# pandekan/tomography_alignment

Measured on AMD Instinct MI355X. Metric: sirt_iterations_per_sec, higher is better.
Workload: dtype f32

## Files before the change

### tomography_alignment_amd/csrc/kernels_tile_gather.hip.h

```cpp

#define GTX 8
#define GTY 8
#define GROWS 14
#define GPITCH 68
#ifndef GWAVES
#define GWAVES 4
#endif
#ifndef GPX
#define GPX 8
#define GPY 12
#endif

#define G_DPP(V, CTRL) __builtin_amdgcn_update_dpp(0, (V), (CTRL), 0xf, 0xf, true)
__device__ __forceinline__ int gwave_min_i32(int v)
{
    v = min(v, G_DPP(v, 0xB1));
    v = min(v, G_DPP(v, 0x4E));
    v = min(v, G_DPP(v, 0x141));
    v = min(v, G_DPP(v, 0x140));
    return min(min(__builtin_amdgcn_readlane(v, 0), __builtin_amdgcn_readlane(v, 16)), min(__builtin_amdgcn_readlane(v, 32), __builtin_amdgcn_readlane(v, 48)));
}
__device__ __forceinline__ int gwave_max_i32(int v)
{
    v = max(v, G_DPP(v, 0xB1));
// ... 251 lines not shown
    float4 t = {0.f, 0.f, 0.f, 0.f};
    int ix_lo = 0;
    bool hit = false;
    if (n_grp > 0) {
        G_TABLE(rk, 0, rk)
        __syncthreads();
        float4 tn;
        int ix_lo_n = 0;
        bool hit_n;
        float y0v[GROWS], yedge = 0.f;
        G_SETUP(0, 0, 0)
        hit = hit_n;
        if (hit) G_STAGE(0)
        t = tn; ix_lo = ix_lo_n;
    }
    for (int grp = 0; grp < n_grp; ++grp) {
        const int nbuf = buf == 2 ? 0 : buf + 1;
        if (grp + 1 < n_grp) G_TABLE((grp + 1) * nl + rk, nbuf, rk)
        __syncthreads();
        const int g0 = grp * nl, g1 = min(n_proj, g0 + nl);
        for (int ip = g0; ip < g1; ++ip) {
            float4 tn = t;
            int ix_lo_n = ix_lo;
            bool hit_n = false;
            float y0v[GROWS], yedge = 0.f;
            const bool more = ip + 1 < n_proj;
            if (more) {
                const bool same = ip + 1 < g1;
                const int sbuf = same ? buf : nbuf, sslot = same ? ip + 1 - g0 : 0;
                G_SETUP(ip + 1, sbuf, sslot)
            }
            if (hit) {
                const int i0 = __builtin_bit_cast(int, t.x);
                const float W0 = t.y, W1 = t.z, W2 = t.w;
                const int slot0 = min(max(i0 - ix_lo, 0), GROWS - 3);
                const float4 *q = (const float4 *)__builtin_assume_aligned(wrows + slot0 * GPITCH, 16);
                float4 n0 = q[0], n1 = q[GPITCH / 4], n2 = q[2 * GPITCH / 4];
#pragma unroll
                for (int p = 0; p < 64; p += 4) {
                    const float4 r0 = n0, r1 = n1, r2 = n2;
                    if (p + 4 < 64) { n0 = q[(p + 4) / 4]; n1 = q[(GPITCH + p + 4) / 4]; n2 = q[(2 * GPITCH + p + 4) / 4]; }
                    acc2[p / 2] = W2 * f32x2{r2.x, r2.y} + (W1 * f32x2{r1.x, r1.y} + (W0 * f32x2{r0.x, r0.y} + acc2[p / 2]));
                    acc2[p / 2 + 1] = W2 * f32x2{r2.z, r2.w} + (W1 * f32x2{r1.z, r1.w} + (W0 * f32x2{r0.z, r0.w} + acc2[p / 2 + 1]));
                    __builtin_amdgcn_sched_barrier(0);
                }
            }
            hit = hit_n;
            if (hit) G_STAGE(ip + 1)
            t = tn; ix_lo = ix_lo_n;
        }
        buf = nbuf;
    }
#undef G_TABLE
#undef G_ROW_LOAD
#undef G_SETUP
#undef G_ZLERP
#undef G_STAGE
#undef G_HIT
    if (UPD) {
        if (X < xe && Y < g.ny) {
            const size_t o = ((size_t)X * g.ny + Y) * g.nz + z0;
            gather_update_store<false>(vol + o, upd_v + o, upd_gt ? upd_gt + o : nullptr, acc2, z0, g.nz, positivity, upd_err);
        }
    } else if (zlive && X < xe && Y < g.ny) {
        float *dst = vol + ((size_t)X * g.ny + Y) * g.nz + z0;
        if (z0 + 64 <= g.nz && (g.nz & 3) == 0) {
#pragma unroll
            for (int p = 0; p < 64; p += 4) {
                float4 v = *(float4 *)(dst + p);
                v.x += acc2[p / 2].x; v.y += acc2[p / 2].y; v.z += acc2[p / 2 + 1].x; v.w += acc2[p / 2 + 1].y;
                *(float4 *)(dst + p) = v;
            }
        } else {
#pragma unroll
            for (int p = 0; p < 64; ++p)
                if (z0 + p < g.nz) dst[p] += (p & 1) ? acc2[p / 2].y : acc2[p / 2].x;
        }
    }
}


#define FGROWS 24
#define FG_NONE (1 << 29)

template <int NW, int WALKY>
__device__ __forceinline__ void fwd_gather_flat_body(const GfC *__restrict__ cs, const int *__restrict__ perm, int n_list, unsigned block_id,
                                                     float *__restrict__ proj, const float *__restrict__ vol, const TomoGeomC &g,
                                                     const unsigned char *__restrict__ vflags, const int *__restrict__ zshift,
                                                     float (*rows)[FGROWS * GPITCH], float4 (*wtab)[GWAVES][64], int (*ltab)[GWAVES][64], int *wlive)
{
    static_assert(NW == 3 || NW == 4, "NW");
    constexpr int SW = FGROWS - NW + 1;
    const int lane = threadIdx.x & 63;
    const int wv = __builtin_amdgcn_readfirstlane(threadIdx.x >> 6);
    const int nS = WALKY ? g.ny : g.nx, nL = WALKY ? g.nx : g.ny;
    const uint32_t strideL4 = (WALKY ? (uint32_t)g.ny * (uint32_t)g.nz : (uint32_t)g.nz) * 4u;
    const size_t strideS = WALKY ? (size_t)g.nz : (size_t)g.ny * g.nz;
    const int npg = (n_list + 7) / 8, nrt = (g.ndx + 7) / 8, nzq = (g.nz + 64 * GWAVES - 1) / (64 * GWAVES) + 1;
    const int m_all = npg * nrt, m8 = (m_all + 7) / 8;
    const int slot_id = (int)(block_id >> 3), xcd = (int)(block_id & 7);
    const int zq = slot_id / m8, tile = xcd * m8 + slot_id % m8;
    if (tile >= m_all || zq >= nzq) return;
    const int pg = tile / nrt, rt = tile % nrt;
    const int z0 = (zq * GWAVES + wv - *zshift) * 64;
    bool zlive = z0 >= 0 && z0 < g.nz;
    if (zlive) {
        const int i = z0 + lane;
        zlive = __builtin_amdgcn_ballot_w64(i < g.nz && vflags[i] != 0) != 0;
    }
    if (lane == 0) wlive[wv] = zlive ? 1 : 0;
    __syncthreads();
    int nl = 0, rk = 0;
#pragma unroll
    for (int w = 0; w < GWAVES; ++w) { nl += wlive[w]; rk += w < wv ? wlive[w] : 0; }
#if !defined(__gfx950__) && !defined(__gfx942__) && !defined(__gfx90a__) && defined(__HIP_DEVICE_COMPILE__)
#error "k_fwd_gather_flat: divergent exit before barriers is only known to be safe on gfx9-family targets (s_barrier ignores ended waves)"
#endif
    if (!zlive) return;

    const int ipl = pg * 8 + (lane >> 3), ix = rt * 8 + (lane & 7);
    const int pe = perm[min(ipl, n_list - 1)];
    const bool ray_ok = ipl < n_list && ix < g.ndx && pe >= 0;
    const GfC &c = cs[max(pe, 0)];
    const int64_t fds = WALKY ? c.fdy : c.fdx, fdl = WALKY ? c.fdx : c.fdy;
    const int64_t bs0 = (WALKY ? c.fp0y : c.fp0x) + (int64_t)ix * (WALKY ? c.fuy : c.fux);
    const int64_t bl0 = (WALKY ? c.fp0x : c.fp0y) + (int64_t)ix * (WALKY ? c.fux : c.fuy);
    const float bsf = (float)((double)bs0 * 2.3283064365386963e-10), inv_ds = (float)(4294967296.0 / (double)fds);
    const int n_smp = ray_ok ? c.n : 0;
    const float two_m32 = 2.3283064365386963e-10f;
    const int Zl = z0 + lane;
    const unsigned long long mz = __builtin_amdgcn_ballot_w64(Zl < g.nz);
    const uint32_t o0 = (uint32_t)min(Zl, g.nz - 1) * 4u;
    float *wrows = rows[wv];
    f32x2 acc2[32];
#pragma unroll
    for (int p = 0; p < 32; ++p) acc2[p] = f32x2{0.f, 0.f};

    int s_lo, s_hi;
    {
        const float dsf = (float)((double)fds * 2.3283064365386963e-10), dlf = (float)((double)fdl * 2.3283064365386963e-10);
        const float blf = (float)((double)bl0 * 2.3283064365386963e-10);
        float ja = 0.f, jb = (float)(n_smp - 1);
        if (fabsf(dlf) > 1e-6f) {
            const float ta = (-1.05f - blf) / dlf, tb = ((float)nL + 0.05f - blf) / dlf;
            ja = fmaxf(ja, fminf(ta, tb) - 2.f);
            jb = fminf(jb, fmaxf(ta, tb) + 2.f);
        } else if (!(blf > -1.5f && blf < (float)nL + 0.5f))
            jb = -1.f;
        int lo = FG_NONE, hi = -FG_NONE;
        if (ja <= jb) {
            const float pa = bsf + ja * dsf, pb = bsf + jb * dsf, top = (float)nS + 4.f;
            lo = (int)floorf(fminf(fmaxf(fminf(pa, pb), -4.f), top)) - 2;
            hi = (int)ceilf(fminf(fmaxf(fmaxf(pa, pb), -4.f), top)) + 3;
        }
        s_lo = max(__builtin_amdgcn_readfirstlane(gwave_min_i32(lo)), 0);
        s_hi = min(__builtin_amdgcn_readfirstlane(gwave_max_i32(hi)), nS);
    }
    if (s_lo >= s_hi) return;

#define FG_TABLE(SX, BUF, SLOT)                                                                                            \
    {                                                                                                                      \
        float W[4] = {0.f, 0.f, 0.f, 0.f};                                                                                 \
        int L0 = FG_NONE;                                                                                                  \
        if ((SX) < s_hi) {                                                                                                 \
            const float ta = ((float)((SX) - 1) - bsf) * inv_ds, tb = ((float)((SX) + 1) - bsf) * inv_ds;                  \
            const int j0 = (int)ceilf(fminf(ta, tb) - 5e-3f);                                                              \
            int64_t sx = bs0 + (int64_t)j0 * fds - ((int64_t)(SX) << 32), sl = bl0 + (int64_t)j0 * fdl;                    \
            float wx[3], fl[3];                                                                                            \
            int hl[3];                                                                                                     \
            _Pragma("unroll") for (int mth = 0; mth < 3; ++mth) {                                                          \
                const int hx = (int)(sx >> 32);                                                                            \
                const float fx = (float)(unsigned)sx * two_m32;                                                            \
                float w = hx == -1 ? fx : (hx == 0 ? 1.f - fx : 0.f);                                                      \
                w = (unsigned)(j0 + mth) < (unsigned)n_smp ? w : 0.f;                                                      \
                wx[mth] = w;                                                                                               \
                hl[mth] = (int)(sl >> 32);                                                                                 \
                fl[mth] = (float)(unsigned)sl * two_m32;                                                                   \
                if (w > 0.f) L0 = min(L0, hl[mth]);                                                                        \
                sx += fds; sl += fdl;                                                                                      \
            }                                                                                                              \
            _Pragma("unroll") for (int mth = 0; mth < 3; ++mth) {                                                          \
                const int rel = hl[mth] - L0;                                                                              \
                const float wl1 = wx[mth] * fl[mth], wl0 = wx[mth] - wl1;                                                  \
                _Pragma("unroll") for (int k = 0; k < NW; ++k) W[k] += rel == k ? wl0 : (rel == k - 1 ? wl1 : 0.f);        \
            }                                                                                                              \
            bool any = false;                                                                                              \
            _Pragma("unroll") for (int k = 0; k < NW; ++k) {                                                               \
                W[k] = (unsigned)(L0 + k) < (unsigned)nL ? W[k] : 0.f;                                                     \
                any |= W[k] != 0.f;                                                                                        \
            }                                                                                                              \
            if (!any) L0 = FG_NONE;                                                                                        \
        }                                                                                                                  \
        wtab[BUF][SLOT][lane] = make_float4(W[0], W[1], W[2], W[3]);                                                       \
        ltab[BUF][SLOT][lane] = L0;                                                                                        \
    }
    const uint32_t slab_bytes = (uint32_t)min(WALKY ? (unsigned long long)(g.nx - 1) * strideL4 + (unsigned long long)g.nz * 4ull
                                                    : (unsigned long long)g.ny * g.nz * 4ull, 0xffffffffull);
#define FG_SLAB_RSRC(SX) __builtin_amdgcn_make_buffer_rsrc((void *)(vol + (size_t)(SX) * strideS), 0, (int)slab_bytes, 0x00020000)
#define FG_LINE_LOAD(RS, SOFF) __builtin_bit_cast(float, __builtin_amdgcn_raw_buffer_load_b32((RS), o0, (SOFF), 0))
#define FG_SETUP(SX, BUF, SLOT)                                                                                            \
    {                                                                                                                      \
        tn = wtab[BUF][SLOT][lane];                                                                                        \
        Ln = ltab[BUF][SLOT][lane];                                                                                        \
        Llo_n = __builtin_amdgcn_readfirstlane(gwave_min_i32(Ln));                                                         \
        Lhi_n = __builtin_amdgcn_readfirstlane(gwave_max_i32(Ln == FG_NONE ? -FG_NONE : Ln));                              \
        need_n = 0;                                                                                                        \
        if (Llo_n != FG_NONE) {                                                                                            \
            const __amdgpu_buffer_rsrc_t srs = FG_SLAB_RSRC(SX);                                                           \
            const uint32_t lineoff = (uint32_t)min(max(Llo_n + min(lane, FGROWS - 1), 0), nL - 1) * strideL4;              \
                    \
            need_n = min(Lhi_n - Llo_n + NW, FGROWS);                                                                      \
            _Pragma("unroll") for (int r4 = 0; r4 < FGROWS; r4 += 4)                                                       \
                if (r4 < need_n) {                                                                                         \
                    _Pragma("unroll") for (int r = r4; r < r4 + 4; ++r)                                                    \
                        yv[r] = FG_LINE_LOAD(srs, (uint32_t)__builtin_amdgcn_readlane((int)lineoff, r));                   \
                }                                                                                                          \
        }                                                                                                                  \
    }
#define FG_STAGE                                                                                                           \
    {                                                                                                                      \
        if (mz == ~0ull) {                                                                                                 \
            _Pragma("unroll") for (int r4 = 0; r4 < FGROWS; r4 += 4)                                                       \
                if (r4 < need_n) {                                                                                         \
                    _Pragma("unroll") for (int r = r4; r < r4 + 4; ++r) wrows[r * GPITCH + lane] = yv[r];                  \
                }                                                                                                          \
        } else {                                                                                                           \
            _Pragma("unroll") for (int r4 = 0; r4 < FGROWS; r4 += 4)                                                       \
                if (r4 < need_n) {                                                                                         \
                    _Pragma("unroll") for (int r = r4; r < r4 + 4; ++r) wrows[r * GPITCH + lane] = select_lanes(yv[r], mz); \
                }                                                                                                          \
        }                                                                                                                  \
    }
#define FG_ACCUM(LBASE)                                                                                                    \
    {                                                                                                                      \
        const int rel = L - (LBASE);                                                                                       \
        const bool inw = (unsigned)rel < (unsigned)SW;                                                                     \
        const int slot0 = inw ? rel : 0;                                                                                   \
        const float W0 = inw ? t.x : 0.f, W1 = inw ? t.y : 0.f, W2 = inw ? t.z : 0.f, W3 = inw ? t.w : 0.f;                \
        const float4 *q = (const float4 *)__builtin_assume_aligned(wrows + slot0 * GPITCH, 16);                            \
        float4 n0 = q[0], n1 = q[GPITCH / 4], n2 = q[2 * GPITCH / 4], n3 = {0.f, 0.f, 0.f, 0.f};                           \
        if (NW == 4) n3 = q[3 * GPITCH / 4];                                                                               \
        _Pragma("unroll") for (int p = 0; p < 64; p += 4) {                                                                \
            const float4 r0 = n0, r1 = n1, r2 = n2, r3 = n3;                                                               \
            if (p + 4 < 64) {                                                                                              \
                n0 = q[(p + 4) / 4]; n1 = q[(GPITCH + p + 4) / 4]; n2 = q[(2 * GPITCH + p + 4) / 4];                       \
                if (NW == 4) n3 = q[(3 * GPITCH + p + 4) / 4];                                                             \
            }                                                                                                              \
            f32x2 a = W2 * f32x2{r2.x, r2.y} + (W1 * f32x2{r1.x, r1.y} + (W0 * f32x2{r0.x, r0.y} + acc2[p / 2]));          \
            f32x2 b = W2 * f32x2{r2.z, r2.w} + (W1 * f32x2{r1.z, r1.w} + (W0 * f32x2{r0.z, r0.w} + acc2[p / 2 + 1]));      \
            if (NW == 4) { a = W3 * f32x2{r3.x, r3.y} + a; b = W3 * f32x2{r3.z, r3.w} + b; }                               \
            acc2[p / 2] = a; acc2[p / 2 + 1] = b;                                                                          \
            __builtin_amdgcn_sched_barrier(0);                                                                             \
        }                                                                                                                  \
    }
    const int n_grp = (s_hi - s_lo + nl - 1) / nl;
    int buf = 0;
    FG_TABLE(s_lo + rk, 0, rk)
    __syncthreads();
    float4 t;
    int L, Llo, Lhi;
    {
        float4 tn;
        int Ln, Llo_n, Lhi_n, need_n;
        float yv[FGROWS];
        FG_SETUP(s_lo, 0, 0)
        FG_STAGE
        t = tn; L = Ln; Llo = Llo_n; Lhi = Lhi_n;
    }
    for (int grp = 0; grp < n_grp; ++grp) {
        const int nbuf = buf == 2 ? 0 : buf + 1;
        if (grp + 1 < n_grp) FG_TABLE(s_lo + (grp + 1) * nl + rk, nbuf, rk)
        __syncthreads();
        const int g0 = s_lo + grp * nl, g1 = min(s_hi, g0 + nl);
        for (int sx = g0; sx < g1; ++sx) {
            float4 tn = t;
            int Ln = L, Llo_n = FG_NONE, Lhi_n = 0, need_n = 0;
            float yv[FGROWS];
            if (sx + 1 < s_hi) {
                const bool same = sx + 1 < g1;
                const int sbuf = same ? buf : nbuf, sslot = same ? sx + 1 - g0 : 0;
                FG_SETUP(sx + 1, sbuf, sslot)
            }
            if (Llo != FG_NONE) {
                FG_ACCUM(Llo)
                for (int lb = Llo + SW; lb <= Lhi; lb += SW) {
                    const __amdgpu_buffer_rsrc_t srs = FG_SLAB_RSRC(sx);
                    for (int r = 0; r < FGROWS; r += 4) {
                        float e[4];
#pragma unroll
                        for (int k = 0; k < 4; ++k) e[k] = FG_LINE_LOAD(srs, (uint32_t)min(max(lb + r + k, 0), nL - 1) * strideL4);
#pragma unroll
                        for (int k = 0; k < 4; ++k) wrows[(r + k) * GPITCH + lane] = select_lanes(e[k], mz);
                    }
                    FG_ACCUM(lb)
                }
            }
            FG_STAGE
            t = tn; L = Ln; Llo = Llo_n; Lhi = Lhi_n;
        }
        buf = nbuf;
    }
#undef FG_TABLE
#undef FG_SLAB_RSRC
#undef FG_LINE_LOAD
#undef FG_SETUP
#undef FG_STAGE
#undef FG_ACCUM
    if (!ray_ok) return;
    const int iz0 = z0 - c.zc;
    float *dst = proj + (size_t)c.slot * ((size_t)g.ndx * g.ndz) + (size_t)ix * g.ndz + iz0;
    const float tau = c.tau;
    if (tau == 0.f) {
        if (iz0 >= 0 && iz0 + 64 <= g.ndz && ((iz0 | g.ndz) & 3) == 0) {
#pragma unroll
            for (int p = 0; p < 64; p += 4) *(float4 *)(dst + p) = make_float4(acc2[p / 2].x, acc2[p / 2].y, acc2[p / 2 + 1].x, acc2[p / 2 + 1].y);
        } else {
#pragma unroll
            for (int p = 0; p < 64; ++p)
                if ((unsigned)(iz0 + p) < (unsigned)g.ndz) dst[p] = (p & 1) ? acc2[p / 2].y : acc2[p / 2].x;
        }
    } else {
        const float wfz = 1.f - tau;
#define FG_S(P) (((P) & 1) ? acc2[(P) / 2].y : acc2[(P) / 2].x)
#pragma unroll
        for (int p = 0; p < 63; ++p)
            if ((unsigned)(iz0 + p) < (unsigned)g.ndz) dst[p] = wfz * FG_S(p) + tau * FG_S(p + 1);
        if ((unsigned)(iz0 + 63) < (unsigned)g.ndz) atomicAdd(dst + 63, wfz * FG_S(63));
        if ((unsigned)(iz0 - 1) < (unsigned)g.ndz) atomicAdd(dst - 1, tau * FG_S(0));
#undef FG_S
    }
}

__global__ __launch_bounds__(GWAVES * 64, 3) void k_fwd_gather_flat(const GfC *__restrict__ cs, const int *__restrict__ perm, int n0, int n1, int n2, int n3,
                                                                    float *__restrict__ proj, const float *__restrict__ vol, TomoGeomC g,
                                                                    const unsigned char *__restrict__ vflags, const int *__restrict__ zshift)
{
    __shared__ __attribute__((aligned(16))) float rows[GWAVES][FGROWS * GPITCH];
    __shared__ float4 wtab[3][GWAVES][64];
    __shared__ int ltab[3][GWAVES][64];
    __shared__ int wlive[GWAVES];
    const unsigned nrt = (unsigned)(g.ndx + 7) / 8, nzq = (unsigned)(g.nz + 64 * GWAVES - 1) / (64 * GWAVES) + 1;
    const unsigned w0 = 8u * ((((unsigned)n0 + 7) / 8 * nrt + 7) / 8) * nzq, w1 = 8u * ((((unsigned)n1 + 7) / 8 * nrt + 7) / 8) * nzq,
                   w2 = 8u * ((((unsigned)n2 + 7) / 8 * nrt + 7) / 8) * nzq;
    unsigned b = blockIdx.x;
    if (b < w0) { fwd_gather_flat_body<3, 0>(cs, perm, n0, b, proj, vol, g, vflags, zshift, rows, wtab, ltab, wlive); return; }
    b -= w0;
    if (b < w1) { fwd_gather_flat_body<4, 0>(cs, perm + n0, n1, b, proj, vol, g, vflags, zshift, rows, wtab, ltab, wlive); return; }
    b -= w1;
    if (b < w2) { fwd_gather_flat_body<3, 1>(cs, perm + n0 + n1, n2, b, proj, vol, g, vflags, zshift, rows, wtab, ltab, wlive); return; }
    b -= w2;
    fwd_gather_flat_body<4, 1>(cs, perm + n0 + n1 + n2, n3, b, proj, vol, g, vflags, zshift, rows, wtab, ltab, wlive);
}
```

### tomography_alignment_amd/csrc/tomo_ctx.h

```cpp
#ifndef TOMO_CTX_H_
#define TOMO_CTX_H_
#include <hip/hip_runtime.h>
#include <rccl/rccl.h>

#include <deque>
#include <map>
#include <string>
#include <vector>

#include "../../include/tomo.h"
#include "tomo_raycore.h"

struct BpC {
    float rp[3][3], ra[3][3], rb[3][3];
    float t[3];
};

struct ProfRec { int64_t n = 0; double ms = 0.0; };
struct ProfPending { std::string name; hipEvent_t e0, e1; };

struct TilePlan {
    bool valid = false;
    bool ok = false;
    std::vector<double> poses;
    int opts = 0;
    double weight_bound = 2.0;
    int n_flat = 0, n_gather = 0;
    double eb_max = 0.0;
    int zc_lo = 0, zc_hi = 0;
    size_t gf_off = 0, fg_off = 0;
    int fg_n[4] = {0, 0, 0, 0};
    bool fg_ok = false;
};

struct ZfKey {
    const void *src = nullptr;
    int nproj = 0, ndz = 0, ndx = 0, nz = 0, zc_lo = 0, zc_hi = 0;
    bool operator==(const ZfKey &o) const
    {
        return src == o.src && nproj == o.nproj && ndz == o.ndz && ndx == o.ndx && nz == o.nz && zc_lo == o.zc_lo && zc_hi == o.zc_hi;
    }
};

struct tomo_ctx {
    int device = 0;
    hipStream_t stream = nullptr;
    bool has_geom = false;
    TomoGeomC g{};
    double vox_pitch[3] = {1, 1, 1};
    float *d_volpad = nullptr;
    size_t volpad_elems = 0;
    size_t volpad_rows = 0;
    bool halo_dirty = true;
    bool wide_rows = false;
    const void *staged_src = nullptr;
    int reuse_staged = 0;
    void *h_stage = nullptr;
    void *d_stage = nullptr;
    size_t stage_bytes = 0;
    TilePlan plan;
    double *d_red = nullptr;
    double *h_red = nullptr;
    size_t red_cap = 0;
    int comm_test_copy_eighths = 0, comm_test_copy_wgs = 0;
    void *d_comm_scratch = nullptr;
    size_t comm_scratch_bytes = 0;
    double *d_red_part = nullptr;
    size_t red_part_cap = 0;
    double *d_acc = nullptr;
    double *h_acc = nullptr;
    int *d_blk = nullptr;
    size_t blk_ints = 0;
    int reuse_sino_flags = 0;
    ZfKey zf_key;
    bool zf_has_cum = false, zf_has_shift = false;
    bool zf_recorded = false;
    float *d_ws = nullptr;
    size_t ws_elems = 0;
    void *csr_data = nullptr, *csr_indices = nullptr, *csr_indptr = nullptr;
    int64_t csr_nnz = 0, csr_rows = 0;
    int csr_value_bytes = 4;
    int fwd_variant = 3;
    int adj_variant = 2;
    int grad_variant = 4;
    int grad_v1_prec = 0;
    int tile_flat = 1;
    int fused_update = 1;
    int adj_flat_gather = 1;
    int fwd_flat_gather = 1;
    int fwd_flat_ztiles = 2;
    hipEvent_t ev0 = nullptr, ev1 = nullptr;
    bool profile_on = false;
    std::map<std::string, ProfRec> prof;
    std::vector<ProfPending> pending;
    std::vector<hipEvent_t> ev_pool;
    ncclComm_t comm = nullptr;
    hipStream_t comm_stream = nullptr;
    hipEvent_t ev_compute = nullptr, ev_comm = nullptr;
    bool comm_pending = false;
    std::deque<hipEvent_t> comm_done;
    std::deque<hipEvent_t> comm_done_g;
    int comm_test_poison_us = 0;
    std::vector<hipEvent_t> comm_ev_pool;
    int n_ranks = 1, rank = 0;
    std::string err;
};

int tomo_fail(tomo_ctx *ctx, int code, const std::string &msg);

struct TomoRange {
    bool on;
    explicit TomoRange(const char *name);
    ~TomoRange();
    TomoRange(const TomoRange &) = delete;
    TomoRange &operator=(const TomoRange &) = delete;
};
int tomo_roctx_enable(int on);
int tomo_ensure_stage(tomo_ctx *ctx, size_t bytes);
int tomo_ensure_red(tomo_ctx *ctx, size_t n_doubles);
int tomo_ensure_red_part(tomo_ctx *ctx, size_t n_doubles);
int tomo_ensure_ws(tomo_ctx *ctx, size_t n_floats);
int tomo_ensure_blk(tomo_ctx *ctx, size_t n_ints);
struct BlkHead {
    unsigned char *zf;
    int *zcum, *zshift;
    size_t ints;
};
static inline int tomo_blk_head(tomo_ctx *ctx, size_t extra_ints, BlkHead *h)
{
    const size_t zf_ints = ((size_t)ctx->g.ndz + 3) / 4;
    h->ints = zf_ints + (size_t)ctx->g.ndz + 2;
    const int rc = tomo_ensure_blk(ctx, h->ints + extra_ints);
    if (rc) return rc;
    h->zf = (unsigned char *)ctx->d_blk;
    h->zcum = ctx->d_blk + zf_ints;
    h->zshift = h->zcum + ctx->g.ndz + 1;
    return TOMO_OK;
}
struct LiveList {
    int *list;
    unsigned char *flags;
    static size_t ints(size_t n) { return 1 + n + (n + 3) / 4; }
    LiveList(int *d_blk, size_t at, size_t n) : list(d_blk + at), flags((unsigned char *)(list + 1 + n)) {}
};
int tomo_record_zflags(tomo_ctx *ctx, const void *d_proj, int n_proj, bool want_cum, bool want_shift, const BlkHead &head, const char *prof_name,
                       bool recorded);
void tomo_csr_release(tomo_ctx *ctx);
void tomo_prof_begin(tomo_ctx *ctx, const char *name);
void tomo_prof_end(tomo_ctx *ctx);
void tomo_prof_begin_on(tomo_ctx *ctx, const char *name, hipStream_t stream);
void tomo_prof_end_on(tomo_ctx *ctx, hipStream_t stream);

#define TOMO_HIP(ctx, call)                                                                         \
    do {                                                                                            \
        hipError_t e_ = (call);                                                                     \
        if (e_ != hipSuccess)                                                                       \
            return tomo_fail((ctx), TOMO_ERR_HIP, std::string(#call) + ": " + hipGetErrorString(e_)); \
    } while (0)

#define TOMO_NEED_GEOM(ctx)                                                              \
    do {                                                                                 \
        if (!(ctx)) return tomo_fail(nullptr, TOMO_ERR_ARG, "null ctx");                 \
        if (!(ctx)->has_geom) return tomo_fail((ctx), TOMO_ERR_STATE, "geometry not set"); \
        {                        \
            hipError_t e_ = hipSetDevice((ctx)->device);                                                         \
            if (e_ != hipSuccess) return tomo_fail((ctx), TOMO_ERR_HIP, std::string("hipSetDevice: ") + hipGetErrorString(e_)); \
        }                                                                                                        \
    } while (0)

#define TOMO_LAUNCH(ctx, name, kern, grid, block, shmem, ...)                                   \
    do {                                                                                        \
// ... 9 lines not shown
```

### tomography_alignment_amd/csrc/tomo_ctx.hip

```cpp
#include <string.h>

#include <algorithm>

#include "tomo_ctx.h"

static std::string g_last_error;

int tomo_fail(tomo_ctx *ctx, int code, const std::string &msg)
{
    g_last_error = msg;
    if (ctx) ctx->err = msg;
    return code;
}

extern "C" int tomo_abi_version(void) { return TOMO_ABI_VERSION; }

extern "C" const char *tomo_last_error(const tomo_ctx *ctx) { return ctx ? ctx->err.c_str() : g_last_error.c_str(); }

extern "C" int tomo_device_count(int *n)
{
    if (!n) return tomo_fail(nullptr, TOMO_ERR_ARG, "null n");
    TOMO_HIP(nullptr, hipGetDeviceCount(n));
    return TOMO_OK;
}
// ... 85 lines not shown
    TOMO_HIP(ctx, hipMemcpyAsync(d, h, bytes, hipMemcpyHostToDevice, ctx->stream));
    TOMO_HIP(ctx, hipStreamSynchronize(ctx->stream));
    return TOMO_OK;
}

extern "C" int tomo_memcpy_d2h(tomo_ctx *ctx, void *h, const void *d, size_t bytes)
{
    if (!ctx) return tomo_fail(ctx, TOMO_ERR_ARG, "null ctx");
    TOMO_HIP(ctx, hipMemcpyAsync(h, d, bytes, hipMemcpyDeviceToHost, ctx->stream));
    TOMO_HIP(ctx, hipStreamSynchronize(ctx->stream));
    return TOMO_OK;
}

extern "C" int tomo_memcpy_d2d(tomo_ctx *ctx, void *dst, const void *src, size_t bytes)
{
    if (!ctx) return tomo_fail(ctx, TOMO_ERR_ARG, "null ctx");
    ctx->zf_recorded = false;
    TOMO_HIP(ctx, hipMemcpyAsync(dst, src, bytes, hipMemcpyDeviceToDevice, ctx->stream));
    return TOMO_OK;
}

extern "C" int tomo_memset0(tomo_ctx *ctx, void *d, size_t bytes)
{
    if (!ctx) return tomo_fail(ctx, TOMO_ERR_ARG, "null ctx");
    ctx->zf_recorded = false;
    TOMO_HIP(ctx, hipMemsetAsync(d, 0, bytes, ctx->stream));
    return TOMO_OK;
}

extern "C" int tomo_sync(tomo_ctx *ctx)
{
    if (!ctx) return tomo_fail(ctx, TOMO_ERR_ARG, "null ctx");
    TOMO_HIP(ctx, hipStreamSynchronize(ctx->stream));
    return TOMO_OK;
}

extern "C" int tomo_ctx_make_current(tomo_ctx *ctx)
{
    if (!ctx) return tomo_fail(ctx, TOMO_ERR_ARG, "null ctx");
    TOMO_HIP(ctx, hipSetDevice(ctx->device));
    return TOMO_OK;
}

extern "C" int tomo_ctx_stream(tomo_ctx *ctx, void **stream)
{
    if (!ctx || !stream) return tomo_fail(ctx, TOMO_ERR_ARG, "tomo_ctx_stream: null argument");
    *stream = reinterpret_cast<void *>(ctx->stream);
    return TOMO_OK;
}

extern "C" int tomo_ctx_set_cu_mask(tomo_ctx *ctx, const uint32_t *mask, int n_words)
{
    if (!ctx || n_words < 0 || (n_words > 0 && !mask)) return tomo_fail(ctx, TOMO_ERR_ARG, "tomo_ctx_set_cu_mask: bad args");
    if (n_words > 0) {
        bool any = false;
        for (int i = 0; i < n_words; ++i) any |= mask[i] != 0;
        if (!any) return tomo_fail(ctx, TOMO_ERR_ARG, "tomo_ctx_set_cu_mask: empty mask (n_words = 0 restores the unrestricted stream)");
    }
    TOMO_HIP(ctx, hipSetDevice(ctx->device));
    TOMO_HIP(ctx, hipStreamSynchronize(ctx->stream));
    hipStream_t s = nullptr;
    if (n_words == 0) TOMO_HIP(ctx, hipStreamCreateWithFlags(&s, hipStreamNonBlocking));
    else TOMO_HIP(ctx, hipExtStreamCreateWithCUMask(&s, (uint32_t)n_words, mask));
    (void)hipStreamDestroy(ctx->stream);
    ctx->stream = s;
    return TOMO_OK;
}

extern "C" int tomo_set_option(tomo_ctx *ctx, const char *key, int value)
{
    if (!ctx || !key) return tomo_fail(ctx, TOMO_ERR_ARG, "bad args");
    if (!strcmp(key, "fwd_variant")) ctx->fwd_variant = value;
    else if (!strcmp(key, "adj_variant")) ctx->adj_variant = value;
    else if (!strcmp(key, "tile_flat")) ctx->tile_flat = value;
    else if (!strcmp(key, "grad_variant")) ctx->grad_variant = value;
    else if (!strcmp(key, "grad_v1_prec")) ctx->grad_v1_prec = value & 3;
    else if (!strcmp(key, "comm_test_poison_us")) ctx->comm_test_poison_us = value;
    else if (!strcmp(key, "comm_test_copy_eighths")) ctx->comm_test_copy_eighths = value < 0 ? 0 : value;
    else if (!strcmp(key, "comm_test_copy_wgs")) ctx->comm_test_copy_wgs = value < 0 ? 0 : value;
    else if (!strcmp(key, "adj_flat_gather")) ctx->adj_flat_gather = value;
    else if (!strcmp(key, "fused_update")) ctx->fused_update = value;
    else if (!strcmp(key, "fwd_flat_ztiles")) ctx->fwd_flat_ztiles = value;
    else if (!strcmp(key, "fwd_flat_gather")) ctx->fwd_flat_gather = value;
    else if (!strcmp(key, "reuse_staged_volume")) ctx->reuse_staged = value;
    else if (!strcmp(key, "reuse_sino_flags")) ctx->reuse_sino_flags = value;
    else if (!strcmp(key, "roctx")) {
        if (tomo_roctx_enable(value)) return tomo_fail(ctx, TOMO_ERR_UNSUPPORTED, "roctx: neither librocprofiler-sdk-roctx.so nor libroctx64.so could be loaded");
    }
    else return tomo_fail(ctx, TOMO_ERR_ARG, std::string("unknown option ") + key);
    return TOMO_OK;
}

int tomo_ensure_stage(tomo_ctx *ctx, size_t bytes)
{
    ctx->plan.valid = false;
    if (bytes <= ctx->stage_bytes) return TOMO_OK;
    TOMO_HIP(ctx, hipStreamSynchronize(ctx->stream));
    if (ctx->d_stage) (void)hipFree(ctx->d_stage);
    if (ctx->h_stage) (void)hipHostFree(ctx->h_stage);
    ctx->d_stage = ctx->h_stage = nullptr;
    ctx->stage_bytes = 0;
    size_t cap = std::max<size_t>(bytes, 1 << 16);
    TOMO_HIP(ctx, hipMalloc(&ctx->d_stage, cap));
    TOMO_HIP(ctx, hipHostMalloc(&ctx->h_stage, cap, hipHostMallocDefault));
    ctx->stage_bytes = cap;
    return TOMO_OK;
}

int tomo_ensure_red(tomo_ctx *ctx, size_t n)
{
    if (n <= ctx->red_cap) return TOMO_OK;
    TOMO_HIP(ctx, hipStreamSynchronize(ctx->stream));
    if (ctx->d_red) (void)hipFree(ctx->d_red);
    if (ctx->h_red) (void)hipHostFree(ctx->h_red);
    ctx->d_red = ctx->h_red = nullptr;
    ctx->red_cap = 0;
    size_t cap = std::max<size_t>(n, 4096);
    TOMO_HIP(ctx, hipMalloc((void **)&ctx->d_red, cap * sizeof(double)));
    TOMO_HIP(ctx, hipHostMalloc((void **)&ctx->h_red, cap * sizeof(double), hipHostMallocDefault));
    ctx->red_cap = cap;
    return TOMO_OK;
}

int tomo_ensure_red_part(tomo_ctx *ctx, size_t n)
{
    if (n <= ctx->red_part_cap) return TOMO_OK;
    TOMO_HIP(ctx, hipStreamSynchronize(ctx->stream));
    if (ctx->d_red_part) (void)hipFree(ctx->d_red_part);
    ctx->d_red_part = nullptr;
    ctx->red_part_cap = 0;
    TOMO_HIP(ctx, hipMalloc((void **)&ctx->d_red_part, n * sizeof(double)));
    ctx->red_part_cap = n;
    return TOMO_OK;
}

extern "C" int tomo_release_workspace(tomo_ctx *ctx)
{
    if (!ctx) return tomo_fail(ctx, TOMO_ERR_ARG, "null ctx");
    TOMO_HIP(ctx, hipSetDevice(ctx->device));
    TOMO_HIP(ctx, hipStreamSynchronize(ctx->stream));
    if (ctx->d_ws) (void)hipFree(ctx->d_ws);
    ctx->d_ws = nullptr;
    ctx->ws_elems = 0;
    if (ctx->d_red_part) (void)hipFree(ctx->d_red_part);
    ctx->d_red_part = nullptr;
    ctx->red_part_cap = 0;
    return TOMO_OK;
}

int tomo_ensure_ws(tomo_ctx *ctx, size_t n)
{
    if (n <= ctx->ws_elems) return TOMO_OK;
    TOMO_HIP(ctx, hipStreamSynchronize(ctx->stream));
    if (ctx->d_ws) (void)hipFree(ctx->d_ws);
    ctx->d_ws = nullptr;
    ctx->ws_elems = 0;
    TOMO_HIP(ctx, hipMalloc((void **)&ctx->d_ws, n * sizeof(float)));
    ctx->ws_elems = n;
    return TOMO_OK;
}

int tomo_ensure_blk(tomo_ctx *ctx, size_t n)
{
    if (n <= ctx->blk_ints) return TOMO_OK;
    ctx->zf_key.src = nullptr;
    TOMO_HIP(ctx, hipStreamSynchronize(ctx->stream));
// ... 724 lines not shown
```

### tomography_alignment_amd/csrc/tomo_project.hip

```cpp
#include <limits.h>
#include <string.h>

#include <algorithm>
#include <climits>
#include <vector>

#include "tomo_ctx.h"

#include "kernels_ray.hip.h"
#include "kernels_tile.hip.h"
#include "kernels_tile_flat.hip.h"
#include "kernels_tile_gather.hip.h"
#include "kernels_grad.hip.h"

static inline bool grad_pose_is_tilted(const ProjC &c) { return fabs(c.w[0]) + fabs(c.w[1]) > 0.0157; }

static int upload_projc(tomo_ctx *ctx, const double *h_poses, int n, bool with_grad, ProjC **d_pc, GradC **d_gc,
                        const int32_t *h_rows = nullptr, int *n_first = nullptr)
{
    const size_t pc_bytes = sizeof(ProjC) * (size_t)n;
    const size_t gc_off = (pc_bytes + 255) & ~(size_t)255;
    const size_t total = gc_off + (with_grad ? sizeof(GradC) * (size_t)n : 0);
    TOMO_HIP(ctx, hipStreamSynchronize(ctx->stream));
    int rc = tomo_ensure_stage(ctx, total);
// ... 115 lines not shown
            q.n = a.n; q.slot = a.slot;
            {
                const bool walky = llabs(q.fdx) < llabs(q.fdy);
                const int64_t ads = llabs(walky ? q.fdy : q.fdx), adl = llabs(walky ? q.fdx : q.fdy);
                p.fg_ok = p.fg_ok && (double)ads >= 0.67 * 4294967296.0 && (double)adl < 0.999 * 4294967296.0;
                std::vector<int> &fl = fg_list[2 * (walky ? 1 : 0) + (2 * adl <= ads ? 0 : 1)];
                if (!fl.empty() && fl.back() != (int)gfc.size() - 1)
                    while (fl.size() % 8) fl.push_back(-1);
                fl.push_back((int)gfc.size());
            }
            gath.push_back(a);
            gfc.push_back(q);
            p.eb_max = std::max(p.eb_max, eb);
            p.zc_lo = std::min(p.zc_lo, (int)q.zc);
            p.zc_hi = std::max(p.zc_hi, (int)q.zc);
        } else
            (untilted ? flat : gen).push_back(a);
    }
    AdjC *h = (AdjC *)ctx->h_stage;
    size_t k = 0;
    for (const AdjC &a : gath) h[k++] = a;
    for (const AdjC &a : flat) h[k++] = a;
    for (const AdjC &a : gen) h[k++] = a;
    GfC *hg = (GfC *)((char *)ctx->h_stage + p.gf_off);
    for (size_t i = 0; i < gfc.size(); ++i) hg[i] = gfc[i];
    int *hf = (int *)((char *)ctx->h_stage + p.fg_off);
    size_t fg_total = 0;
    for (int l = 0; l < 4; ++l) {
        for (int v : fg_list[l]) hf[fg_total++] = v;
        p.fg_n[l] = (int)fg_list[l].size();
    }
    if (n_proj) TOMO_HIP(ctx, hipMemcpyAsync(ctx->d_stage, h, p.fg_off + sizeof(int) * fg_total, hipMemcpyHostToDevice, ctx->stream));
    p.n_gather = (int)gath.size();
    p.n_flat = (int)(gath.size() + flat.size());
    p.poses.assign(h_poses, h_poses + n_pose_doubles);
    p.opts = opts;
    p.ok = p.valid = true;
    return TOMO_OK;
}

static inline const AdjC *plan_adjc(const tomo_ctx *ctx) { return (const AdjC *)ctx->d_stage; }
static inline const GfC *plan_gfc(const tomo_ctx *ctx, const TilePlan &p) { return (const GfC *)((const char *)ctx->d_stage + p.gf_off); }
static inline const int *plan_fwd_lists(const tomo_ctx *ctx, const TilePlan &p) { return (const int *)((const char *)ctx->d_stage + p.fg_off); }

static inline dim3 tile_grid(const TomoGeomC &g, int tz = ATZ) { return dim3((g.nz + 1 + tz - 1) / tz, (g.ny + 1 + ATY - 1) / ATY, (g.nx + 1 + ATX - 1) / ATX); }

static int forward_tiles(tomo_ctx *ctx, const double *h_poses, int n_proj, const float *d_vol, float *d_proj, int xt0, int xt1, bool *done,
                         bool whole = false)
{
    const TomoGeomC &g = ctx->g;
    *done = false;
    if (ctx->fwd_variant != 3 || n_proj <= 0) return TOMO_OK;
    dim3 grid = tile_grid(g);
    if (grid.y > 65535 || grid.z > 65535) return TOMO_OK;
    const TilePlan *plan = nullptr;
    int rc = stage_tile_consts(ctx, h_poses, n_proj, &plan);
    if (rc) return rc;
    if (!plan->ok) return TOMO_OK;
    *done = true;
    xt0 = std::max(xt0, 0);
    xt1 = std::min(xt1, (int)grid.z);
    if (xt1 <= xt0) return TOMO_OK;
    grid.z = (unsigned)(xt1 - xt0);
    const AdjC *d_c = plan_adjc(ctx);
    const int n_flat = plan->n_flat;
    size_t flat_ints = 0;
    ctx->zf_key.src = nullptr;
    if (whole && ctx->fwd_flat_gather && plan->n_gather == n_proj && plan->fg_ok && plan->eb_max < 1.49 &&
        std::max(g.nx, g.ny) <= 8192 && (unsigned long long)g.nx * g.ny * g.nz * 4ull <= (1ull << 32)) {
        const size_t zf_ints = ((size_t)g.nz + 3) / 4;
        rc = tomo_ensure_blk(ctx, zf_ints + 1);
        if (rc) return rc;
        unsigned char *d_vf = (unsigned char *)ctx->d_blk;
        int *d_shift = ctx->d_blk + zf_ints;
        TOMO_HIP(ctx, hipMemsetAsync(d_vf, 0, (size_t)g.nz, ctx->stream));
        const long long n_lines = (long long)g.nx * g.ny;
        TOMO_LAUNCH(ctx, "k_fwd_live", k_sino_zflags, dim3((unsigned)((g.nz + 255) / 256), (unsigned)std::min<long long>(n_lines, 4096)), dim3(256), 0,
                    d_vol, n_lines, g.nz, d_vf);
        TOMO_LAUNCH(ctx, "k_fwd_live", k_zchunk_shift, dim3(1), dim3(64), 0, (const unsigned char *)d_vf, g.nz, g.nz, 0, -1, d_shift);
        const GfC *d_gfc = plan_gfc(ctx, *plan);
        const int *d_perm = plan_fwd_lists(ctx, *plan);
        const int nrt = (g.ndx + 7) / 8, nzq = (g.nz + 64 * GWAVES - 1) / (64 * GWAVES) + 1;
        const int *fn = plan->fg_n;
        long long n_wg = 0;
        for (int l = 0; l < 4; ++l) n_wg += 8 * (((long long)((fn[l] + 7) / 8) * nrt + 7) / 8) * nzq;
        if (n_wg >= ((long long)1 << 31)) return tomo_fail(ctx, TOMO_ERR_UNSUPPORTED, "gather forward: grid too large");
        TOMO_LAUNCH(ctx, "k_fwd_tile_flat", k_fwd_gather_flat, dim3((unsigned)n_wg), dim3(GWAVES * 64), 0, d_gfc, d_perm, fn[0], fn[1], fn[2], fn[3], d_proj, d_vol, g,
                    (const unsigned char *)d_vf, (const int *)d_shift);
        return TOMO_OK;
    }
    if (n_flat > 0) {
        dim3 fg = tile_grid(g, FTZ);
        fg.z = grid.z;
        if (fg.x >= 2 && ctx->fwd_flat_ztiles >= 2) {
            const int nzb = (g.nz + 2 * FLZ - 1) / (2 * FLZ), nty = (int)fg.y;
            const size_t n_blk = (size_t)nzb * nty * fg.z;
            if (n_blk >= (size_t)1 << 30) return tomo_fail(ctx, TOMO_ERR_ARG, "tomo_forward: volume too large for the flat forward's block list");
            flat_ints = LiveList::ints(n_blk);
            rc = tomo_ensure_blk(ctx, flat_ints + (n_proj > n_flat ? LiveList::ints((size_t)grid.x * grid.y * grid.z) : 0));
            if (rc) return rc;
            const LiveList live(ctx->d_blk, 0, n_blk);
            TOMO_LAUNCH(ctx, "k_fwd_live", k_fwd_live, dim3((unsigned)n_blk), dim3(256), 0, d_vol, g, xt0, nzb, nty, live.flags);
            TOMO_LAUNCH(ctx, "k_fwd_live", k_fwd_compact, dim3(1), dim3(1024), 0, live.flags, (int)n_blk, live.list);
            TOMO_LAUNCH(ctx, "k_fwd_tile_flat", k_fwd_flat_tab, dim3((unsigned)n_blk), dim3(FZ_WAVES * 64), 0, d_c, n_flat, d_proj, d_vol, g, xt0,
                        (const int *)live.list, (const unsigned char *)live.flags, nzb, nty);
        }
        else
            TOMO_LAUNCH(ctx, "k_fwd_tile_flat", k_tile_flat<true>, fg, dim3(ADJ_WAVES * 64), 0, d_c, n_flat, d_proj,
                        (float *)d_vol, g, (const unsigned *)nullptr, 1.f, xt0);
    }
    if (n_proj > n_flat) {
        const size_t n_tile = (size_t)grid.x * grid.y * grid.z;
        if (n_tile >= (size_t)1 << 30) return tomo_fail(ctx, TOMO_ERR_ARG, "tomo_forward: volume too large for the tile list");
        rc = tomo_ensure_blk(ctx, flat_ints + LiveList::ints(n_tile));
        if (rc) return rc;
        const LiveList live(ctx->d_blk, flat_ints, n_tile);
        TOMO_LAUNCH(ctx, "k_fwd_live", k_tile_live, dim3((unsigned)n_tile), dim3(256), 0, d_vol, g, xt0, (int)grid.x, (int)grid.y, live.flags);
        TOMO_LAUNCH(ctx, "k_fwd_live", k_fwd_compact, dim3(1), dim3(1024), 0, (const unsigned char *)live.flags, (int)n_tile, live.list);
        TOMO_LAUNCH(ctx, "k_fwd_tile", (k_tile<true, TILE_FWD_WAVES>), dim3((unsigned)n_tile), dim3(TILE_FWD_WAVES * 64), 0, d_c + n_flat, n_proj - n_flat, d_proj, (float *)d_vol,
                    g, (const unsigned *)nullptr, 1.f, xt0, (const int *)live.list, (int)grid.x, (int)grid.y, (const int *)nullptr);
    }
    return TOMO_OK;
}

extern "C" int tomo_forward(tomo_ctx *ctx, const double *h_poses, int n_proj, const float *d_vol, float *d_proj)
{
    TomoRange roctx_range("tomo_forward");
    TOMO_NEED_GEOM(ctx);
    if (!h_poses || !d_vol || !d_proj || n_proj < 0) return tomo_fail(ctx, TOMO_ERR_ARG, "tomo_forward: bad args");
    if (n_proj == 0) return TOMO_OK;
    const TomoGeomC &g = ctx->g;
    const size_t n_det = (size_t)g.ndx * g.ndz;
    int rc;
    if (ctx->fwd_variant == 3) {
        TOMO_HIP(ctx, hipMemsetAsync(d_proj, 0, n_det * (size_t)n_proj * sizeof(float), ctx->stream));
        bool done = false;
        rc = forward_tiles(ctx, h_poses, n_proj, d_vol, d_proj, 0, INT_MAX, &done, true);
        if (rc) return rc;
        if (done) return TOMO_OK;
    }
    rc = stage_volume(ctx, d_vol);
    if (rc) return rc;
    for (int p0 = 0; p0 < n_proj; p0 += TOMO_MAX_GRID_Z) {
        const int np = std::min(TOMO_MAX_GRID_Z, n_proj - p0);
        ProjC *d_pc = nullptr;
        rc = upload_projc(ctx, h_poses + (size_t)p0 * TOMO_POSE_STRIDE, np, false, &d_pc, nullptr);
        if (rc) return rc;
        float *out = d_proj + (size_t)p0 * n_det;
        if (ctx->fwd_variant == 1 || ctx->wide_rows)
            TOMO_LAUNCH(ctx, "k_fwd_v1", k_fwd_v1, ray_grid(g, np), dim3(256), 0, d_pc, ctx->d_volpad, out, g);
        else
            TOMO_LAUNCH(ctx, "k_fwd_v2", k_fwd_v2, ray_grid(g, np), dim3(256), 0, d_pc, ctx->d_volpad, out, g);
    }
    return TOMO_OK;
}

extern "C" int tomo_forward_xslab(tomo_ctx *ctx, const double *h_poses, int n_proj, const float *d_vol, float *d_proj, int xt0, int xt1)
{
    TomoRange roctx_range("tomo_forward_xslab");
    TOMO_NEED_GEOM(ctx);
    if (!h_poses || !d_vol || !d_proj || n_proj < 0 || xt0 < 0 || xt1 < xt0) return tomo_fail(ctx, TOMO_ERR_ARG, "tomo_forward_xslab: bad args");
    bool done = false;
    int rc = forward_tiles(ctx, h_poses, n_proj, d_vol, d_proj, xt0, xt1, &done);
    if (rc) return rc;
    if (!done) return tomo_fail(ctx, TOMO_ERR_UNSUPPORTED, "tomo_forward_xslab: these poses do not take the tile kernels");
    return TOMO_OK;
}

static int adjoint_atomic(tomo_ctx *ctx, const double *h_poses, int n_proj, const float *d_proj, float *d_vol, int accumulate)
{
    const TomoGeomC &g = ctx->g;
// ... 551 lines not shown
```

Baseline: 3.741.

## Group forward gather workgroups into projection/row patches per XCD

Adds a patched block-to-tile mapping for the flat gather forward kernel. Each run of consecutive slot ids on an XCD now covers a 16x4 patch of projection groups and row tiles at one z chunk, instead of striding through the flattened tile list. The goal is that concurrently resident workgroups on one XCD read overlapping volume slabs and so reuse its L2. The patched mapping is on by default once the patch count reaches a threshold, and it can launch extra idle workgroups from partial patches and rounding.

New measurement: 3.899 (median of 6 runs). 1.04x the previous value.

```diff
diff --git a/tomography_alignment_amd/csrc/kernels_tile_gather.hip.h b/tomography_alignment_amd/csrc/kernels_tile_gather.hip.h
--- a/tomography_alignment_amd/csrc/kernels_tile_gather.hip.h
+++ b/tomography_alignment_amd/csrc/kernels_tile_gather.hip.h
@@ -357,10 +357,23 @@
 
 #define FGROWS 24
 #define FG_NONE (1 << 29)
+#ifndef FPG
+#define FPG 16
+#define FPR 4
+#endif
+#define FWD_PATCH_MIN 128
+
+__host__ __device__ static inline unsigned long long fg_list_wgs(int n_list, int nrt, int nzq, int patched)
+{
+    const unsigned long long npg = (unsigned long long)((n_list + 7) / 8);
+    if (!patched) return 8ull * ((npg * (unsigned long long)nrt + 7) / 8) * (unsigned long long)nzq;
+    const unsigned long long npq = ((npg + FPG - 1) / FPG) * (unsigned long long)((nrt + FPR - 1) / FPR);
+    return 8ull * ((npq * (unsigned long long)nzq + 7) / 8) * (unsigned long long)(FPG * FPR);
+}
 
 template <int NW, int WALKY>
 __device__ __forceinline__ void fwd_gather_flat_body(const GfC *__restrict__ cs, const int *__restrict__ perm, int n_list, unsigned block_id,
-                                                     float *__restrict__ proj, const float *__restrict__ vol, const TomoGeomC &g,
+                                                     int patched, float *__restrict__ proj, const float *__restrict__ vol, const TomoGeomC &g,
                                                      const unsigned char *__restrict__ vflags, const int *__restrict__ zshift,
                                                      float (*rows)[FGROWS * GPITCH], float4 (*wtab)[GWAVES][64], int (*ltab)[GWAVES][64], int *wlive)
 {
@@ -372,11 +385,27 @@
     const uint32_t strideL4 = (WALKY ? (uint32_t)g.ny * (uint32_t)g.nz : (uint32_t)g.nz) * 4u;
     const size_t strideS = WALKY ? (size_t)g.nz : (size_t)g.ny * g.nz;
     const int npg = (n_list + 7) / 8, nrt = (g.ndx + 7) / 8, nzq = (g.nz + 64 * GWAVES - 1) / (64 * GWAVES) + 1;
-    const int m_all = npg * nrt, m8 = (m_all + 7) / 8;
     const int slot_id = (int)(block_id >> 3), xcd = (int)(block_id & 7);
-    const int zq = slot_id / m8, tile = xcd * m8 + slot_id % m8;
-    if (tile >= m_all || zq >= nzq) return;
-    const int pg = tile / nrt, rt = tile % nrt;
+    int pg, rt, zq;
+    if (patched) {
+        const int npp = (npg + FPG - 1) / FPG, nrp = (nrt + FPR - 1) / FPR, npq = npp * nrp;
+        const int within = slot_id % (FPG * FPR);
+        const int patch = (slot_id / (FPG * FPR)) * 8 + xcd;
+        zq = patch / npq;
+        const int pgp = (patch % npq) / nrp, rtp = (patch % npq) % nrp;
+        const int pg0 = pgp * npg / npp, pgc = (pgp + 1) * npg / npp - pg0, rt0 = rtp * nrt / nrp, rtc = (rtp + 1) * nrt / nrp - rt0;
+        if (zq >= nzq || within / FPR >= pgc || within % FPR >= rtc) return;
+        pg = pg0 + within / FPR;
+        rt = rt0 + within % FPR;
+    } else {
+        const int m_all = npg * nrt, m8 = (m_all + 7) / 8;
+        const int tile = xcd * m8 + slot_id % m8;
+        zq = slot_id / m8;
+        if (tile >= m_all) return;
+        pg = tile / nrt;
+        rt = tile % nrt;
+    }
+    if (zq >= nzq) return;
     const int z0 = (zq * GWAVES + wv - *zshift) * 64;
     bool zlive = z0 >= 0 && z0 < g.nz;
     if (zlive) {
@@ -471,7 +500,11 @@
     }
     const uint32_t slab_bytes = (uint32_t)min(WALKY ? (unsigned long long)(g.nx - 1) * strideL4 + (unsigned long long)g.nz * 4ull
                                                     : (unsigned long long)g.ny * g.nz * 4ull, 0xffffffffull);
+#ifdef TOMO_ABLATE_FWD_SLAB_LO
+#define FG_SLAB_RSRC(SX) __builtin_amdgcn_make_buffer_rsrc((void *)(vol + (size_t)(s_lo) * strideS), 0, (int)slab_bytes, 0x00020000)
+#else
 #define FG_SLAB_RSRC(SX) __builtin_amdgcn_make_buffer_rsrc((void *)(vol + (size_t)(SX) * strideS), 0, (int)slab_bytes, 0x00020000)
+#endif
 #define FG_LINE_LOAD(RS, SOFF) __builtin_bit_cast(float, __builtin_amdgcn_raw_buffer_load_b32((RS), o0, (SOFF), 0))
 #define FG_SETUP(SX, BUF, SLOT)                                                                                            \
     {                                                                                                                      \
@@ -607,22 +640,22 @@
 }
 
 __global__ __launch_bounds__(GWAVES * 64, 3) void k_fwd_gather_flat(const GfC *__restrict__ cs, const int *__restrict__ perm, int n0, int n1, int n2, int n3,
-                                                                    float *__restrict__ proj, const float *__restrict__ vol, TomoGeomC g,
+                                                                    int patched, float *__restrict__ proj, const float *__restrict__ vol, TomoGeomC g,
                                                                     const unsigned char *__restrict__ vflags, const int *__restrict__ zshift)
 {
     __shared__ __attribute__((aligned(16))) float rows[GWAVES][FGROWS * GPITCH];
     __shared__ float4 wtab[3][GWAVES][64];
     __shared__ int ltab[3][GWAVES][64];
     __shared__ int wlive[GWAVES];
-    const unsigned nrt = (unsigned)(g.ndx + 7) / 8, nzq = (unsigned)(g.nz + 64 * GWAVES - 1) / (64 * GWAVES) + 1;
-    const unsigned w0 = 8u * ((((unsigned)n0 + 7) / 8 * nrt + 7) / 8) * nzq, w1 = 8u * ((((unsigned)n1 + 7) / 8 * nrt + 7) / 8) * nzq,
-                   w2 = 8u * ((((unsigned)n2 + 7) / 8 * nrt + 7) / 8) * nzq;
+    const int nrt = (g.ndx + 7) / 8, nzq = (g.nz + 64 * GWAVES - 1) / (64 * GWAVES) + 1;
+    const unsigned w0 = (unsigned)fg_list_wgs(n0, nrt, nzq, patched), w1 = (unsigned)fg_list_wgs(n1, nrt, nzq, patched),
+                   w2 = (unsigned)fg_list_wgs(n2, nrt, nzq, patched);
     unsigned b = blockIdx.x;
-    if (b < w0) { fwd_gather_flat_body<3, 0>(cs, perm, n0, b, proj, vol, g, vflags, zshift, rows, wtab, ltab, wlive); return; }
+    if (b < w0) { fwd_gather_flat_body<3, 0>(cs, perm, n0, b, patched, proj, vol, g, vflags, zshift, rows, wtab, ltab, wlive); return; }
     b -= w0;
-    if (b < w1) { fwd_gather_flat_body<4, 0>(cs, perm + n0, n1, b, proj, vol, g, vflags, zshift, rows, wtab, ltab, wlive); return; }
+    if (b < w1) { fwd_gather_flat_body<4, 0>(cs, perm + n0, n1, b, patched, proj, vol, g, vflags, zshift, rows, wtab, ltab, wlive); return; }
     b -= w1;
-    if (b < w2) { fwd_gather_flat_body<3, 1>(cs, perm + n0 + n1, n2, b, proj, vol, g, vflags, zshift, rows, wtab, ltab, wlive); return; }
+    if (b < w2) { fwd_gather_flat_body<3, 1>(cs, perm + n0 + n1, n2, b, patched, proj, vol, g, vflags, zshift, rows, wtab, ltab, wlive); return; }
     b -= w2;
-    fwd_gather_flat_body<4, 1>(cs, perm + n0 + n1 + n2, n3, b, proj, vol, g, vflags, zshift, rows, wtab, ltab, wlive);
-}
+    fwd_gather_flat_body<4, 1>(cs, perm + n0 + n1 + n2, n3, b, patched, proj, vol, g, vflags, zshift, rows, wtab, ltab, wlive);
+}
diff --git a/tomography_alignment_amd/csrc/tomo_ctx.h b/tomography_alignment_amd/csrc/tomo_ctx.h
--- a/tomography_alignment_amd/csrc/tomo_ctx.h
+++ b/tomography_alignment_amd/csrc/tomo_ctx.h
@@ -87,6 +87,7 @@
     int tile_flat = 1;
     int fused_update = 1;
     int adj_flat_gather = 1;
+    int fwd_gather_patch = 1;
     int fwd_flat_gather = 1;
     int fwd_flat_ztiles = 2;
     hipEvent_t ev0 = nullptr, ev1 = nullptr;
diff --git a/tomography_alignment_amd/csrc/tomo_ctx.hip b/tomography_alignment_amd/csrc/tomo_ctx.hip
--- a/tomography_alignment_amd/csrc/tomo_ctx.hip
+++ b/tomography_alignment_amd/csrc/tomo_ctx.hip
@@ -191,6 +191,10 @@
     else if (!strcmp(key, "fused_update")) ctx->fused_update = value;
     else if (!strcmp(key, "fwd_flat_ztiles")) ctx->fwd_flat_ztiles = value;
     else if (!strcmp(key, "fwd_flat_gather")) ctx->fwd_flat_gather = value;
+    else if (!strcmp(key, "fwd_gather_patch")) {
+        if (value < 0 || value > 2) return tomo_fail(ctx, TOMO_ERR_ARG, "fwd_gather_patch: 0, 1 or 2");
+        ctx->fwd_gather_patch = value;
+    }
     else if (!strcmp(key, "reuse_staged_volume")) ctx->reuse_staged = value;
     else if (!strcmp(key, "reuse_sino_flags")) ctx->reuse_sino_flags = value;
     else if (!strcmp(key, "roctx")) {
diff --git a/tomography_alignment_amd/csrc/tomo_project.hip b/tomography_alignment_amd/csrc/tomo_project.hip
--- a/tomography_alignment_amd/csrc/tomo_project.hip
+++ b/tomography_alignment_amd/csrc/tomo_project.hip
@@ -221,11 +221,14 @@
         const int *d_perm = plan_fwd_lists(ctx, *plan);
         const int nrt = (g.ndx + 7) / 8, nzq = (g.nz + 64 * GWAVES - 1) / (64 * GWAVES) + 1;
         const int *fn = plan->fg_n;
-        long long n_wg = 0;
-        for (int l = 0; l < 4; ++l) n_wg += 8 * (((long long)((fn[l] + 7) / 8) * nrt + 7) / 8) * nzq;
-        if (n_wg >= ((long long)1 << 31)) return tomo_fail(ctx, TOMO_ERR_UNSUPPORTED, "gather forward: grid too large");
-        TOMO_LAUNCH(ctx, "k_fwd_tile_flat", k_fwd_gather_flat, dim3((unsigned)n_wg), dim3(GWAVES * 64), 0, d_gfc, d_perm, fn[0], fn[1], fn[2], fn[3], d_proj, d_vol, g,
-                    (const unsigned char *)d_vf, (const int *)d_shift);
+        long long n_patch = 0;
+        for (int l = 0; l < 4; ++l) n_patch += (long long)(((fn[l] + 7) / 8 + FPG - 1) / FPG) * ((nrt + FPR - 1) / FPR) * nzq;
+        const int patched = ctx->fwd_gather_patch == 2 || (ctx->fwd_gather_patch == 1 && n_patch >= FWD_PATCH_MIN) ? 1 : 0;
+        unsigned long long n_wg = 0;
+        for (int l = 0; l < 4; ++l) n_wg += fg_list_wgs(fn[l], nrt, nzq, patched);
+        if (n_wg >= (1ull << 31)) return tomo_fail(ctx, TOMO_ERR_UNSUPPORTED, "gather forward: grid too large");
+        TOMO_LAUNCH(ctx, patched ? "k_fwd_tile_flat(patched)" : "k_fwd_tile_flat", k_fwd_gather_flat, dim3((unsigned)n_wg), dim3(GWAVES * 64), 0, d_gfc, d_perm, fn[0], fn[1], fn[2], fn[3], patched, d_proj,
+                    d_vol, g, (const unsigned char *)d_vf, (const int *)d_shift);
         return TOMO_OK;
     }
     if (n_flat > 0) {
```
